# andrewcsmith/soundsym

Hardware: AMD Instinct MI355X
Metric: segment-pairs/sec (DTW cost+argmin) (higher is better)
Workload: dtype f32

## Files before the change

### soundsym_amd/csrc/dtw_filter.hip

```cpp
#include "ssym_internal.hpp"
#include "dtw_filter_kernel.hpp"
#include "dtw_filter_wg_kernel.hpp"
#include "dtw_filter_pk_kernel.hpp"
#include "dtw_filter_sp_kernel.hpp"
#include "dtw_band_kernel.hpp"

#include <algorithm>
#include <atomic>
#include <cmath>
#include <cstdlib>

namespace ssym {

static std::atomic<unsigned long long> g_filter_wg_launches{0};

int filter_pieces(int dim)
{
    static const bool k48 = ssym_knob("SSYM_FILTER_K48") != nullptr;
    return dim > kFilterMaxDim2 ? 1 : (k48 ? 2 : 3);
}

__global__ void build_filter_records_kernel(const double *__restrict__ raw, const uint64_t *__restrict__ off,
                                            const uint32_t *__restrict__ perm, uint32_t n, uint32_t dim,
                                            uint32_t dimUse, uint32_t frames_pad, int is_source,
                                            int lead, int pieces, double scale, _Float16 *__restrict__ rec,
                                            unsigned *__restrict__ resid)
{
    const uint32_t s = blockIdx.y;
    const uint32_t seg = perm[s];
    const uint32_t slot = blockIdx.x * blockDim.x + threadIdx.x;
    if (slot >= frames_pad)
        return;
    _Float16 out[kFilterRecHalfs];
#pragma unroll
    for (int i = 0; i < kFilterRecHalfs; ++i)
        out[i] = (_Float16)0.0f;
    const uint32_t nf = seg < n ? (uint32_t)(off[seg + 1] - off[seg]) : 0u;
    const uint32_t first = lead < 0 ? frames_pad - nf : (uint32_t)lead;
    const bool real = slot >= first && slot < first + nf;
    const uint32_t f = slot - first;
    const int nbase = pieces == 3 ? 28 : (pieces == 2 ? 3 : 1) * (int)dimUse;
    const int npieces = pieces == 3 ? 2 : 3;
    if (!real && is_source)
        out[filter_slot_offset(nbase)] = (_Float16)__builtin_inff();
    if (real) {
        const double *p = raw + (off[seg] + f) * dim;
        double nrm = 0.0, res2 = 0.0;
        for (uint32_t e = 0; e < dimUse; ++e) {
            const double v = p[e] * scale;
            const _Float16 h1 = (_Float16)v;
            const bool two = pieces == 2 || (pieces == 3 && (is_source || e < 2));
            const _Float16 h2 = two ? (_Float16)(v - (double)h1) : (_Float16)0.0f;
            const double vh = (double)h1 + (double)h2;
            nrm += vh * vh;
            res2 += (v - vh) * (v - vh);
            const _Float16 m1 = (_Float16)(-2.0f * (float)h1), m2 = (_Float16)(-2.0f * (float)h2);
            if (pieces == 2) {
                out[filter_slot_offset(3 * e + 0)] = is_source ? m1 : h1;
                out[filter_slot_offset(3 * e + 1)] = is_source ? m1 : h2;
                out[filter_slot_offset(3 * e + 2)] = is_source ? m2 : h1;
            } else if (pieces == 3) {
                out[filter_slot_offset(2 * e + 0)] = is_source ? m1 : h1;
                out[filter_slot_offset(2 * e + 1)] = is_source ? m2 : h1;
                if (e < 2)
                    out[filter_slot_offset(26 + e)] = is_source ? m1 : h2;
            } else {
                out[filter_slot_offset(e)] = is_source ? m1 : h1;
            }
        }
        const float r = __double2float_ru(sqrt(res2) / scale * 1.0000001);
        if (r > 0.0f)
            atomicMax(&resid[s], __float_as_uint(r));
        const _Float16 p1 = (_Float16)nrm;
        const _Float16 p2 = (_Float16)(nrm - (double)p1);
        const _Float16 p3 = (_Float16)(nrm - (double)p1 - (double)p2);
        const int mine = nbase + (is_source ? 0 : npieces), other = nbase + (is_source ? npieces : 0);
        out[filter_slot_offset(mine + 0)] = p1;
        out[filter_slot_offset(mine + 1)] = p2;
        out[filter_slot_offset(other + 0)] = (_Float16)1.0f;
        out[filter_slot_offset(other + 1)] = (_Float16)1.0f;
        if (npieces == 3) {
            out[filter_slot_offset(mine + 2)] = p3;
            out[filter_slot_offset(other + 2)] = (_Float16)1.0f;
        }
    }
    if (is_source) {
        _Float16 *dst = rec + ((size_t)s * frames_pad + slot) * kFilterRecHalfs;
#pragma unroll
        for (int i = 0; i < kFilterRecHalfs; ++i)
            dst[i] = out[i];
    } else {
#pragma unroll
        for (int h = 0; h < 2; ++h)
#pragma unroll
            for (int m = 0; m < kFilterKM; ++m) {
                _Float16 *dst = rec + tgt_rec_offset(s, frames_pad, slot, m, h);
#pragma unroll
                for (int i = 0; i < 8; ++i)
                    dst[i] = out[h * 24 + m * 8 + i];
            }
    }
}

static uint32_t band_slots(int radius, const SegmentSet &src, const SegmentSet &tgt)
{
    const uint32_t kb = (uint32_t)(2 * radius + 1 + 15) / 16 * 16;
    return std::max<uint32_t>(radius + src.max_frames, std::max<uint32_t>(tgt.max_frames, 1) + kb) + 1;
}
static size_t band_lds_bytes(int radius, const SegmentSet &src, const SegmentSet &tgt)
{
    return ((size_t)2 * band_slots(radius, src, tgt) * kFilterRecHalfs + kBandImagePad) * sizeof(_Float16);
}

bool filter_band_as_bound(const ssym_ctx *ctx, const SegmentSet &src, const SegmentSet &tgt)
{
    if (ctx->band < 0)
        return false;
    return 2 * ctx->band + 1 > 6 * 16 || band_lds_bytes(ctx->band, src, tgt) > 160 * 1024 - 64;
}

bool filter_supported(const ssym_ctx *ctx, const SegmentSet &src, const SegmentSet &tgt)
{
    if (src.light || tgt.light)
        return false;
    if (src.dim != tgt.dim)
        return false;
    if ((ctx->band < 0 || filter_band_as_bound(ctx, src, tgt)) && filter_shape((int)src.max_frames).nt == 0)
        return false;
    if (!std::isfinite(src.max_abs) || !std::isfinite(tgt.max_abs))
        return false;
    if (!std::isfinite(src.max_sqnorm_all) || !std::isfinite(tgt.max_sqnorm_all))
        return false;
    return src.n > 0 && tgt.n > 0;
}

static double common_scale(const SegmentSet &src, const SegmentSet &tgt)
{
    const double m = std::max(src.max_abs, tgt.max_abs);
    if (!(m > 0.0))
        return 1.0;
    int e = 0;
    (void)std::frexp(m, &e);
    e = std::min(std::max(6 - e, -100), 100);
    const double sq = std::max(src.max_sqnorm_all, tgt.max_sqnorm_all);
    while (e > -200 && sq * std::ldexp(1.0, 2 * e) * 1.01 >= 65000.0)
        --e;
    const double ideal = std::ldexp(1.0, e);
    if (src.rec && src.rec_scale > 0.0 && src.rec_scale <= ideal && src.rec_scale * 16.0 >= ideal)
        return src.rec_scale;
    return ideal;
}

static int32_t ensure_records(ssym_ctx *ctx, const SegmentSet &set, double scale, uint32_t slots, int lead)
{
    const size_t bytes = (size_t)set.n_pad * slots * kFilterRecHalfs * sizeof(_Float16);
    if (set.rec && set.rec_scale == scale && set.rec_bytes == bytes && set.rec_slots == slots &&
        set.rec_lead == lead)
        return SSYM_OK;
    if (set.rec && set.rec_bytes != bytes) {
        dev_free(ctx, set.rec);
        set.rec = nullptr;
    }
    if (!set.rec) {
        int32_t rca = dev_alloc(ctx, &set.rec, bytes);
        if (rca != SSYM_OK)
            return rca;
    }
    set.rec_bytes = bytes;
    dim3 grid((slots + 63) / 64, set.n_pad);
    const int dimUse = filter_dim_used((int)set.dim);
    unsigned *resid = (unsigned *)(set.max_sqnorm + 2 * (size_t)set.n_pad);
    SSYM_HIP_CHECK(ctx, hipMemsetAsync(resid, 0, sizeof(unsigned) * set.n_pad, ctx->stream));
    build_filter_records_kernel<<<grid, 64, 0, ctx->stream>>>(set.raw, set.off, set.perm, set.n, set.dim,
                                                              (uint32_t)dimUse, slots, set.is_source ? 1 : 0, lead,
                                                              filter_pieces(dimUse), scale,
                                                              (_Float16 *)set.rec, resid);
    SSYM_HIP_CHECK(ctx, hipGetLastError());
    set.rec_scale = scale;
    set.rec_slots = slots;
    set.rec_lead = lead;
    return SSYM_OK;
}

static FilterKnobs read_filter_knobs()
{
    FilterKnobs k;
    if (!ssym_knob("SSYM_TEST_HOOKS"))
        return k;
    auto num = [](const char *name, int unset) {
        const char *v = ssym_knob(name);
        return v ? atoi(v) : unset;
    };
    k.pk = num("SSYM_FILTER_PK", 0) != 0;
    k.sp = num("SSYM_FILTER_SP", 1) != 0;
    const int mp = num("SSYM_SP_MULTIPAIR", 1);
    k.spMultipair = mp == 0 || mp == 2 ? mp : 1;
    k.spPairBlock = ssym_knob("SSYM_SP_PAIRBLOCK") ? std::max(num("SSYM_SP_PAIRBLOCK", 0), 0) : -1;
    k.wg = num("SSYM_FILTER_WG", k.wg) != 0;
    k.skip0 = num("SSYM_FILTER_SKIP0", 1) != 0;
    k.nt8 = ssym_knob("SSYM_FILTER_NT8") != nullptr;
    k.oneLaunch = ssym_knob("SSYM_FILTER_ONE_LAUNCH") != nullptr;
    k.longClasses = num("SSYM_FILTER_LONG_CLASSES", 1) != 0;
    k.pruneNt = num("SSYM_PRUNE_NT", 0);
    return k;
}

static const std::vector<uint32_t> &plan_lens(const SegmentSet &set, uint32_t group)
{
    if (set.plan_lens.size() != set.n_pad / group) {
        set.plan_lens.assign(set.n_pad / group, 0u);
        for (uint32_t slot = 0; slot < set.n; ++slot) {
            const uint32_t s = set.h_perm[slot];
            uint32_t &m = set.plan_lens[slot / group];
            m = std::max(m, (uint32_t)(set.h_off[s + 1] - set.h_off[s]));
        }
    }
    return set.plan_lens;
}

struct FilterCall {
    hipStream_t st;
    const SegmentSet &src, &tgt;
    bool sq;
    int ku;
    float outScale;
    float *handoff;
    unsigned *taskCtr;
    float *cmat;
    const float *abandon;
    unsigned long long *colCtr;
    const uint32_t *candSlot;
};

template <int NT, bool SQ, int KU>
static bool run_kernel(const FilterCall &c, const FilterLaunch &l)
{
    constexpr int OCC = NT == 1 ? 3 : NT == 8 ? 1 : 2;
    const dim3 grid(l.grid), block(64 * kFilterWavesPerBlock);
    const _Float16 *srec = (const _Float16 *)c.src.rec, *trec = (const _Float16 *)c.tgt.rec;
    const int rowsPad = (int)c.src.frames_pad, colsPad = (int)c.tgt.frames_pad, tgtPad = (int)c.tgt.n_pad;
    const int nSrcPairs = l.hi - l.lo, nTasks = nSrcPairs * (tgtPad / 32);
    unsigned *ctr = c.taskCtr + l.ctrSet * 8 * kTaskCtrStride;
    switch (l.kind) {
    case FilterKernel::Mp:
        if constexpr (NT == 1) {
            dtw_filter_sp_kernel<KU == 2 ? 3 : 2, SQ, 2, KU, kSpRowBlock, true><<<grid, block, 0, c.st>>>(
                srec, trec, c.src.len, c.tgt.len, rowsPad, colsPad, tgtPad, l.taskPairs, nSrcPairs, l.taskChunk, c.outScale,
                ctr, c.cmat, l.origin, l.lo, l.pairBlock);
            return true;
        }
        return false;
    case FilterKernel::Sp:
        if constexpr (NT <= 3 && (KU == 2 || NT <= 2)) {
            constexpr int OCCSP = (NT == 1 && KU == 2) ? 3 : (NT == 2 && KU == 2) ? SSYM_SP_OCC_NT2 : 2;
            dtw_filter_sp_kernel<NT, SQ, OCCSP, KU, kSpRowBlock><<<grid, block, 0, c.st>>>(
                srec, trec, c.src.len, c.tgt.len, rowsPad, colsPad, tgtPad, nSrcPairs, nTasks, l.taskChunk, c.outScale, ctr,
                c.cmat, l.origin, l.lo, l.pairBlock);
            return true;
        }
        return false;
    case FilterKernel::GenericSkip0:
        if constexpr (NT == 3 || NT == 4) {
            dtw_filter_kernel<NT, SQ, OCC, false, KU, true><<<grid, block, 0, c.st>>>(
                srec, trec, c.src.len, c.tgt.len, rowsPad, l.passes, colsPad, tgtPad, nSrcPairs, nTasks, l.taskChunk,
                c.outScale, c.handoff, ctr, c.cmat, nullptr, nullptr, nullptr, l.origin, l.lo);
            return true;
        }
        return false;
    case FilterKernel::Wg:
        if constexpr (NT == 4) {
            dtw_filter_wg_kernel<SQ, KU><<<grid, block, 0, c.st>>>(
                srec, trec, c.src.len, c.tgt.len, rowsPad, l.passes, colsPad, tgtPad, nSrcPairs / 4, l.taskChunk, c.outScale,
                c.handoff, ctr, c.cmat, l.origin, l.lo);
            g_filter_wg_launches.fetch_add(1, std::memory_order_relaxed);
            return true;
        }
        return false;
    case FilterKernel::Pk:
        if constexpr (NT == 4) {
            dtw_filter_pk_kernel<SQ, KU><<<grid, block, 0, c.st>>>(
                srec, trec, c.src.len, c.tgt.len, rowsPad, l.passes, colsPad, tgtPad, nSrcPairs, nTasks, l.taskChunk,
                c.outScale, c.handoff, ctr, c.cmat, l.origin, l.lo);
            return true;
        }
        return false;
    case FilterKernel::GenericPrune:
        dtw_filter_kernel<NT, SQ, OCC, true, KU><<<grid, block, 0, c.st>>>(
            srec, trec, c.src.len, c.tgt.len, rowsPad, l.passes, colsPad, tgtPad, nSrcPairs, nTasks, l.taskChunk, c.outScale,
            c.handoff, ctr, c.cmat, c.abandon, c.colCtr, c.candSlot, l.origin, l.lo);
        return true;
    case FilterKernel::Generic:
        dtw_filter_kernel<NT, SQ, OCC, false, KU><<<grid, block, 0, c.st>>>(
            srec, trec, c.src.len, c.tgt.len, rowsPad, l.passes, colsPad, tgtPad, nSrcPairs, nTasks, l.taskChunk, c.outScale,
            c.handoff, ctr, c.cmat, nullptr, nullptr, nullptr, l.origin, l.lo);
        return true;
    }
    return false;
}

template <int NT>
static bool run_tiles(const FilterCall &c, const FilterLaunch &l)
{
    if (c.sq)
        return c.ku == 2 ? run_kernel<NT, true, 2>(c, l) : run_kernel<NT, true, 3>(c, l);
    return c.ku == 2 ? run_kernel<NT, false, 2>(c, l) : run_kernel<NT, false, 3>(c, l);
}

static bool run_launch(const FilterCall &c, const FilterLaunch &l)
{
    switch (l.nt) {
    case 1: return run_tiles<1>(c, l);
    case 2: return run_tiles<2>(c, l);
    case 3: return run_tiles<3>(c, l);
    case 4: return run_tiles<4>(c, l);
    case 8: return run_tiles<8>(c, l);
    }
    return false;
}

template <int NTB, int WB, int OCC, bool SQ, int LASTN, bool PRUNE>
static int32_t launch_band_cfg2(ssym_ctx *ctx, const SegmentSet &src, const SegmentSet &tgt, uint32_t slots,
                                size_t lds, float outScale, float *cmat, const float *abandon,
                                unsigned long long *colCtr, const uint32_t *candSlot)
{
    const int nTgtBlocks = (int)tgt.n_pad / (32 * WB);
    const int nTasks = ((int)src.n_pad / 2) * nTgtBlocks;
    const int grid = std::max(1, std::min(ctx->num_cus, nTasks));
    int32_t rc = ensure(ctx, ctx->handoff, 8 * sizeof(unsigned));
    if (rc != SSYM_OK)
        return rc;
    unsigned *taskCtr = (unsigned *)ctx->handoff.ptr;
    rc = zero_words(ctx, taskCtr, sizeof(unsigned));
    if (rc != SSYM_OK)
        return rc;
    const bool two = filter_mfmas(filter_pieces(filter_dim_used((int)src.dim)), filter_dim_used((int)src.dim)) == 2;
    auto kern = two ? dtw_band_kernel<NTB, WB, OCC, SQ, LASTN, PRUNE, 2> : dtw_band_kernel<NTB, WB, OCC, SQ, LASTN, PRUNE, 3>;
#ifdef SSYM_BAND_PAIRCOLS_BUILD
    if constexpr (!PRUNE && LASTN == 1 && NTB >= 4 && OCC == 2) {
        const char *pc = ssym_knob("SSYM_BAND_PAIRCOLS");
        if (pc && atoi(pc) != 0)
            kern = two ? dtw_band_kernel<NTB, WB, OCC, SQ, LASTN, PRUNE, 2, true> : dtw_band_kernel<NTB, WB, OCC, SQ, LASTN, PRUNE, 3, true>;
    }
#endif
    if (lds > 64 * 1024)
        SSYM_HIP_CHECK(ctx, hipFuncSetAttribute((const void *)kern, hipFuncAttributeMaxDynamicSharedMemorySize, (int)lds));
    kern<<<dim3(grid), 64 * WB, lds, ctx->stream>>>(
        (const _Float16 *)src.rec, (const _Float16 *)tgt.rec, src.len, tgt.len, (int)slots, ctx->band,
        (int)tgt.frames_pad, (int)tgt.n_pad, nTgtBlocks, nTasks, taskCtr, outScale, cmat, abandon, colCtr, candSlot);
    SSYM_HIP_CHECK(ctx, hipGetLastError());
    return SSYM_OK;
}

template <int NTB, int WB, int OCC, bool SQ, int LASTN>
static int32_t launch_band_cfg(ssym_ctx *ctx, const SegmentSet &src, const SegmentSet &tgt, uint32_t slots,
                               size_t lds, float outScale, float *cmat, const float *abandon,
                               unsigned long long *colCtr, const uint32_t *candSlot)
{
    return abandon ? launch_band_cfg2<NTB, WB, OCC, SQ, LASTN, true>(ctx, src, tgt, slots, lds, outScale, cmat, abandon, colCtr, candSlot)
                   : launch_band_cfg2<NTB, WB, OCC, SQ, LASTN, false>(ctx, src, tgt, slots, lds, outScale, cmat, nullptr, nullptr, nullptr);
}

template <int NTB, bool SQ>
static int32_t launch_band(ssym_ctx *ctx, const SegmentSet &src, const SegmentSet &tgt, uint32_t slots,
                           size_t lds, float outScale, float *cmat, const float *abandon, unsigned long long *colCtr, const uint32_t *candSlot)
{
    const bool last1 = 2 * ctx->band + 1 == 16 * (NTB - 1) + 1;
    if constexpr (NTB <= 5)
        return last1 ? launch_band_cfg<NTB, 8, 2, SQ, 1>(ctx, src, tgt, slots, lds, outScale, cmat, abandon, colCtr, candSlot)
                     : launch_band_cfg<NTB, 8, 2, SQ, 16>(ctx, src, tgt, slots, lds, outScale, cmat, abandon, colCtr, candSlot);
    else
        return last1 ? launch_band_cfg<NTB, 4, 1, SQ, 1>(ctx, src, tgt, slots, lds, outScale, cmat, abandon, colCtr, candSlot)
                     : launch_band_cfg<NTB, 4, 1, SQ, 16>(ctx, src, tgt, slots, lds, outScale, cmat, abandon, colCtr, candSlot);
}

static int32_t launch_dtw_filter_banded(ssym_ctx *ctx, const SegmentSet &src, const SegmentSet &tgt, float *cmat,
                                        const float *abandon, unsigned long long *colCtr, const uint32_t *candSlot)
{
    if (tgt.n_pad % kBandTgtQuantum != 0 || src.n_pad % 2 != 0) {
        ctx->err = "dtw band filter: segment set not padded for the banded kernel";
        return SSYM_E_UNSUPPORTED;
    }
    const uint32_t slots = band_slots(ctx->band, src, tgt);
    const size_t lds = band_lds_bytes(ctx->band, src, tgt);
    const double scale = common_scale(src, tgt);
    int32_t rc = ensure_records(ctx, src, scale, slots, ctx->band);
    if (rc != SSYM_OK)
        return rc;
    rc = ensure_records(ctx, tgt, scale, tgt.frames_pad, 0);
    if (rc != SSYM_OK)
        return rc;
    const bool sq = ctx->squared != 0;
    const float outScale = (float)(sq ? 1.0 / (scale * scale) : 1.0 / scale);
    const int ntb = (2 * ctx->band + 1 + 15) / 16;
#define SSYM_BCASE(N_)                                                                                  \
    case N_:                                                                                            \
        return sq ? launch_band<N_, true>(ctx, src, tgt, slots, lds, outScale, cmat, abandon, colCtr, candSlot)   \
                  : launch_band<N_, false>(ctx, src, tgt, slots, lds, outScale, cmat, abandon, colCtr, candSlot);
    switch (ntb) {
        SSYM_BCASE(1) SSYM_BCASE(2) SSYM_BCASE(3) SSYM_BCASE(4) SSYM_BCASE(5) SSYM_BCASE(6)
    default:
        ctx->err = "dtw band filter: band radius too large";
        return SSYM_E_UNSUPPORTED;
    }
#undef SSYM_BCASE
}

int32_t ensure_filter_records(ssym_ctx *ctx, const SegmentSet &src, const SegmentSet &tgt, double *scale_out)
{
    const double scale = common_scale(src, tgt);
    int32_t rc = ctx->band >= 0 && !filter_band_as_bound(ctx, src, tgt)
                     ? ensure_records(ctx, src, scale, band_slots(ctx->band, src, tgt), ctx->band)
                     : ensure_records(ctx, src, scale, src.frames_pad, -1);
    if (rc == SSYM_OK)
        rc = ensure_records(ctx, tgt, scale, tgt.frames_pad, 0);
    if (scale_out)
        *scale_out = scale;
    return rc;
}

int32_t launch_dtw_filter(ssym_ctx *ctx, const SegmentSet &src, const SegmentSet &tgt, float *cmat,
                          const float *abandon, unsigned long long *colCtr, const uint32_t *candSlot)
{
    ctx->filter_launches = 1;
    if (ctx->band >= 0 && !filter_band_as_bound(ctx, src, tgt))
        return launch_dtw_filter_banded(ctx, src, tgt, cmat, abandon, colCtr, candSlot);
    const FilterShape shape = filter_shape((int)src.max_frames);
    if (shape.nt == 0 || (int)src.frames_pad != shape.rows() || src.n_pad % 8 != 0 || tgt.n_pad % 32 != 0) {
        ctx->err = "dtw filter: segment set not padded for the filter kernel";
        return SSYM_E_UNSUPPORTED;
    }
    if (((size_t)tgt.frames_pad + 3) / 4 * 1024 >= ((size_t)1 << 31)) {
        ctx->err = "dtw filter: targets too long for the hand-off rows";
        return SSYM_E_UNSUPPORTED;
    }
    const double scale = common_scale(src, tgt);
    int32_t rc = ensure_records(ctx, src, scale, src.frames_pad, -1);
    if (rc != SSYM_OK)
        return rc;
    rc = ensure_records(ctx, tgt, scale, tgt.frames_pad, 0);
    if (rc != SSYM_OK)
        return rc;
    const int gridBlocks = std::max(8, ctx->num_cus * 2 / 8 * 8);
    const size_t handBytes = (size_t)(gridBlocks / 2 * 3) * kFilterWavesPerBlock * ((tgt.frames_pad + 3) / 4) * 256 * sizeof(float);
    const size_t ctrBytes = 8 * kTaskCtrStride * sizeof(unsigned);
    rc = ensure(ctx, ctx->handoff, handBytes + kMaxClasses * ctrBytes);
    if (rc != SSYM_OK)
        return rc;
    unsigned *taskCtr = (unsigned *)((char *)ctx->handoff.ptr + handBytes);
    rc = zero_words(ctx, taskCtr, kMaxClasses * ctrBytes);
    if (rc != SSYM_OK)
        return rc;
    const bool sq = ctx->squared != 0;
    const int dimUse = filter_dim_used((int)src.dim);

    FilterPlanInput in;
    in.pairLen = plan_lens(src, 2).data(), in.groupCols = plan_lens(tgt, 32).data();
    in.srcN = src.n, in.srcNPad = src.n_pad, in.framesPad = src.frames_pad;
    in.tgtN = tgt.n, in.tgtGroups = tgt.n_pad / 32, in.tgtTotalFrames = tgt.total_frames;
    in.numCus = ctx->num_cus;
    in.ku = filter_mfmas(filter_pieces(dimUse), dimUse);
    in.abandon = abandon != nullptr;
    in.pruneSwept = ctx->prune_swept;
    in.knobs = read_filter_knobs();
    const std::vector<FilterLaunch> plan = plan_filter(in);

    ctx->filter_launches = (int)plan.size();
    ctx->launched_cells = 0;
    for (const FilterLaunch &l : plan)
        ctx->launched_cells += l.cells;
    const FilterCall call{ctx->stream, src, tgt, sq, in.ku, (float)(sq ? 1.0 / (scale * scale) : 1.0 / scale),
                          (float *)ctx->handoff.ptr, taskCtr, cmat, abandon, colCtr, candSlot};
    for (const FilterLaunch &l : plan)
        if (!run_launch(call, l)) {
            ctx->err = "dtw filter: the plan names a kernel that is not built";
            return SSYM_E_UNSUPPORTED;
        }
    SSYM_HIP_CHECK(ctx, hipGetLastError());
    return SSYM_OK;
}

}

extern "C" __attribute__((visibility("default"))) unsigned long long ssym_debug_filter_wg_launches(void)
{
    return ssym::g_filter_wg_launches.load(std::memory_order_relaxed);
}

#ifdef SSYM_SP_PROF
extern "C" __attribute__((visibility("default"))) int ssym_debug_sp_prof(unsigned long long *out)
{
    unsigned long long zero[12] = {0, 0, 0, 0, 0, 0, 0, 0, 0, 0, 0, 0};
    if (hipMemcpyFromSymbol(out, HIP_SYMBOL(ssym::ssym_sp_prof), sizeof(zero)) != hipSuccess)
        return -1;
    return hipMemcpyToSymbol(HIP_SYMBOL(ssym::ssym_sp_prof), zero, sizeof(zero)) == hipSuccess ? 0 : -1;
}
#endif
```

### soundsym_amd/csrc/dtw_filter_wg_kernel.hpp

```cpp
#pragma once
#include "dtw_filter_kernel.hpp"

namespace ssym {

#define SSYM_FILTER_SBASE(P_) asm volatile("" : "+s"(P_))
#define SSYM_FILTER_LANEOFF(V_) asm volatile("" : "+v"(V_))

constexpr int kFilterWgRing = 16;
constexpr int kFilterWgLds = kFilterWgRing * kFilterSlotBytes + kFilterWavesPerBlock * kFilterTopBytes;

template <bool SQ, int KU>
__global__ __launch_bounds__(64 * kFilterWavesPerBlock, 2) void dtw_filter_wg_kernel(
    const _Float16 *__restrict__ srcRec, const _Float16 *__restrict__ tgtRec,
    const int *__restrict__ srcLen, const int *__restrict__ tgtLen, int srcRows, int nPasses,
    int tgtFramesPad, int mPad, int nSrcBlocks, int taskChunk, float outScale,
    float *__restrict__ handoff, unsigned *__restrict__ taskCtr, float *__restrict__ cmat,
    int rowOrigin, int spBase)
{
    static_assert(KU == 2 || KU == 3, "two or three operand planes per column");
    static_assert(kFilterWavesPerBlock == 4, "a column group is one column per wave");
    constexpr int NT = 4;
    constexpr int REC = kFilterRecHalfs;
    constexpr int BR = NT * 16;
    const float INF = __builtin_inff();

    const int lane = threadIdx.x & 63;
    const int wave = __builtin_amdgcn_readfirstlane(threadIdx.x >> 6);
    const int col = lane & 31;
    const int half = lane >> 5;
    const size_t handGroups = ((size_t)tgtFramesPad + 3) / 4;
    char *const handRow = reinterpret_cast<char *>(handoff + ((size_t)blockIdx.x * kFilterWavesPerBlock + wave) * handGroups * 256);
    uint32_t laneOff16 = lane * 16;
    const __amdgpu_buffer_rsrc_t handBuf = __builtin_amdgcn_make_buffer_rsrc(handRow, 0, (int)(handGroups * 1024), 0x00020000);
    constexpr int kWaitStaged = wait_vmcnt(KU), kWaitStagedStores = wait_vmcnt(KU + 4);
    __shared__ __attribute__((aligned(16))) char lds[kFilterWgLds];
    char *const ring = lds;
    char *const myTop = lds + kFilterWgRing * kFilterSlotBytes + wave * kFilterTopBytes;
    volatile unsigned *const taskWord = reinterpret_cast<volatile unsigned *>(lds + kFilterWgRing * kFilterSlotBytes);
    unsigned fetches = 0;

    const unsigned nGroups = (unsigned)mPad >> 5;
    for (unsigned hop = 0; hop < 8; ++hop) {
      const unsigned xcd = (blockIdx.x + hop) & 7u;
      const unsigned rangeLen = xcd < nGroups ? ((nGroups - xcd + 7u) >> 3) * (unsigned)nSrcBlocks : 0u;
      for (;;) {
        if (wave == 0) {
            __builtin_amdgcn_s_waitcnt(wait_vmcnt(0));
            asm volatile("" ::: "memory");
            if (lane == 0)
                taskWord[fetches & 1u] = atomicAdd(&taskCtr[xcd * kTaskCtrStride], (unsigned)taskChunk);
        }
        __syncthreads();
        const unsigned got = (unsigned)__builtin_amdgcn_readfirstlane((int)taskWord[fetches & 1u]);
        ++fetches;
        if (got >= rangeLen)
            break;
        const unsigned gotEnd = min(got + (unsigned)taskChunk, rangeLen);
        int preFa = 0, preFb = 0;
        bool havePre = false;
       for (unsigned gi = got; gi < gotEnd; ++gi) {
        const unsigned lin = rangeLen - 1u - gi;
        const int tg = (int)(xcd + 8u * (lin / (unsigned)nSrcBlocks));
        const int sp = spBase + 4 * (int)(lin % (unsigned)nSrcBlocks) + wave;

        const int fa = havePre ? preFa : srcLen[2 * sp + half];
        const int fb_m1 = (havePre ? preFb : tgtLen[32 * tg + col]) - 1;
        havePre = gi + 1 < gotEnd;
        if (havePre) {
            const unsigned linN = lin - 1u;
            preFa = srcLen[2 * (spBase + 4 * (int)(linN % (unsigned)nSrcBlocks) + wave) + half];
            preFb = tgtLen[32 * (int)(xcd + 8u * (linN / (unsigned)nSrcBlocks)) + col];
        }
        const int r0 = srcRows - fa;

        int nCols = fb_m1 + 1;
#pragma unroll
        for (int o = 32; o >= 1; o >>= 1)
            nCols = max(nCols, __shfl_xor(nCols, o));
        nCols = __builtin_amdgcn_readfirstlane(nCols);

        float res = INF;
        const char *const tgtGroup = reinterpret_cast<const char *>(tgtRec) + (size_t)tg * tgtFramesPad * (kTgtFrameHalfs * 2);

        for (int pass = nCols > 0 ? 0 : nPasses; pass < nPasses; ++pass) {
            const int rowBase = rowOrigin + pass * BR;
            int haveTop = pass, passesLeft = nPasses - 1 - pass;
            asm volatile("" : "+s"(haveTop), "+s"(passesLeft));

            auto stage = [&](int gr) {
                const int c = 4 * gr + wave;
                const int cc = min(c, nCols - 1);
                char *slot = ring + (c & (kFilterWgRing - 1)) * kFilterSlotBytes;
                const char *gb = tgtGroup + (size_t)(unsigned)cc * (kTgtFrameHalfs * 2);
                SSYM_FILTER_SBASE(gb);
                SSYM_FILTER_LANEOFF(laneOff16);
                const __attribute__((address_space(1))) void *gp =
                    (const __attribute__((address_space(1))) void *)(gb + laneOff16);
                __attribute__((address_space(3))) void *lp = (__attribute__((address_space(3))) void *)slot;
                __builtin_amdgcn_global_load_lds(gp, lp, 16, 0, 0);
                __builtin_amdgcn_global_load_lds(gp, lp, 16, 1024, 0);
                if (KU == 3)
                    __builtin_amdgcn_global_load_lds(gp, lp, 16, 2048, 0);
            };
            auto stageTop = [&](int g) {
                const int gg = min(g, (nCols - 1) >> 2);
                __builtin_amdgcn_raw_ptr_buffer_load_lds(handBuf, (__attribute__((address_space(3))) void *)(myTop + (g & 1) * 1024),
                                                         16, laneOff16, gg * 1024, 0, 0);
            };
            auto fetch = [&](int c, half8 (&B)[KU], float &top) {
                const char *slot = ring + (c & (kFilterWgRing - 1)) * kFilterSlotBytes;
#pragma unroll
                for (int m = 0; m < KU; ++m)
                    B[m] = *reinterpret_cast<const half8 *>(slot + m * 1024 + lane * 16);
                top = *reinterpret_cast<const float *>(myTop + ((c >> 2) & 1) * 1024 + (c & 3) * 256 + lane * 4);
            };
            half8 A[NT][KU];
            {
                const int arow = lane & 31;
                const int a_src = 2 * sp + ((arow >> 2) & 1);
                const int a_frm = rowBase + (arow & 3) + 4 * (arow >> 3);
                const _Float16 *abase = srcRec + ((size_t)a_src * srcRows + a_frm) * REC + half * 24;
#pragma unroll
                for (int T = 0; T < NT; ++T)
                    load_rec<KU>(abase + (size_t)T * kFilterRowsPerTile * REC, A[T]);
            }

            asm volatile("" ::: "memory");
            __builtin_amdgcn_s_barrier();
            asm volatile("" ::: "memory");
            if (haveTop)
                stageTop(0);
            stage(0);
            stage(1);

            float L0[BR], L1[BR];
#pragma unroll
            for (int i = 0; i < BR; ++i) {
                L0[i] = (rowBase + i == r0 - 1) ? 0.0f : INF;
                L1[i] = L0[i];
            }
            float prevTop = (rowBase == r0) ? 0.0f : INF;

            half8 B0[KU], B1[KU];
            float topN = INF;
            __builtin_amdgcn_s_waitcnt(kWaitStaged);
            asm volatile("" ::: "memory");
            if (!haveTop) {
                typedef float f32x4 __attribute__((ext_vector_type(4)));
                *reinterpret_cast<f32x4 *>(myTop + lane * 16) = f32x4{INF, INF, INF, INF};
                *reinterpret_cast<f32x4 *>(myTop + 1024 + lane * 16) = f32x4{INF, INF, INF, INF};
            }
            __builtin_amdgcn_s_barrier();
            asm volatile("" ::: "memory");
            fetch(0, B0, topN);
            f32x16 acc = mfma_tile<KU>(A[0], B0);

            for (int j0 = 0; j0 < nCols; j0 += 4) {
                const int g = j0 >> 2;
                stage(g + 2);
                SSYM_FILTER_SBASE(passesLeft);
                if (passesLeft == 0 || j0 == 0)
                    __builtin_amdgcn_s_waitcnt(kWaitStaged);
                else
                    __builtin_amdgcn_s_waitcnt(kWaitStagedStores);
                asm volatile("" ::: "memory");
                __builtin_amdgcn_s_barrier();
                asm volatile("" ::: "memory");
#pragma unroll
                for (int q = 0; q < 4; ++q) {
                    const int j = j0 + q;
                    if (j < nCols) {
                        const float up = topN;
                        const float diag = prevTop;
                        prevTop = up;
                        SSYM_FILTER_SBASE(haveTop);
                        SSYM_FILTER_SBASE(passesLeft);
                        if (q == 3 && haveTop) {
                            if (passesLeft == 0)
                                __builtin_amdgcn_s_waitcnt(wait_vmcnt(0));
                            else
                                __builtin_amdgcn_s_waitcnt(wait_vmcnt(3));
                            asm volatile("" ::: "memory");
                        }
                        if ((q & 1) == 0)
                            fetch(j + 1, B1, topN);
                        else
                            fetch(j + 1, B0, topN);
                        if (q == 0 && haveTop)
                            stageTop(g + 1);
                        float bottom;
                        if ((q & 1) == 0)
                            bottom = dp_column<NT, SQ, KU>(A, B0, B1, acc, up, diag, L0, L1);
                        else
                            bottom = dp_column<NT, SQ, KU>(A, B1, B0, acc, up, diag, L1, L0);
                        SSYM_FILTER_SBASE(passesLeft);
                        if (passesLeft != 0) {
                            __builtin_amdgcn_raw_buffer_store_b32(__float_as_uint(bottom), handBuf, lane * 4, g * 1024 + q * 256, 0);
                        } else {
                            res = (j == fb_m1) ? bottom : res;
                        }
                    }
                }
            }
        }
        cmat[(size_t)(2 * sp + half) * mPad + 32 * tg + col] = res * outScale;
       }
      }
    }
}

#undef SSYM_FILTER_SBASE
#undef SSYM_FILTER_LANEOFF

}
```

Measured before the change: 512.0 million.

## Add two-pass workgroup DTW filter kernel with leader/follower waves via LDS handoff

Adds a new wg2 kernel for two-pass workgroup filter launches. Leader waves compute the top row band and pass each column's bottom value to follower waves through LDS, and the followers compute the second band concurrently in a tick-synchronised pipeline. This replaces the sequential two passes that handed off through a global buffer. A front-end task fetcher and a shared target-staging ring are interleaved into the ticks. The kernel is enabled by default, adds per-tick barriers, and halves the pairs processed per block. An ablation macro is also added to the old kernel.

```diff
diff --git a/soundsym_amd/csrc/dtw_filter.hip b/soundsym_amd/csrc/dtw_filter.hip
--- a/soundsym_amd/csrc/dtw_filter.hip
+++ b/soundsym_amd/csrc/dtw_filter.hip
@@ -1,6 +1,7 @@
 #include "ssym_internal.hpp"
 #include "dtw_filter_kernel.hpp"
 #include "dtw_filter_wg_kernel.hpp"
+#include "dtw_filter_wg2_kernel.hpp"
 #include "dtw_filter_pk_kernel.hpp"
 #include "dtw_filter_sp_kernel.hpp"
 #include "dtw_band_kernel.hpp"
@@ -13,6 +14,8 @@
 namespace ssym {
 
 static std::atomic<unsigned long long> g_filter_wg_launches{0};
+static std::atomic<unsigned long long> g_filter_wg2_launches{0};
+static std::atomic<bool> g_filter_wg2{true};
 
 int filter_pieces(int dim)
 {
@@ -185,6 +188,7 @@
 static FilterKnobs read_filter_knobs()
 {
     FilterKnobs k;
+    g_filter_wg2.store(true, std::memory_order_relaxed);
     if (!ssym_knob("SSYM_TEST_HOOKS"))
         return k;
     auto num = [](const char *name, int unset) {
@@ -197,6 +201,7 @@
     k.spMultipair = mp == 0 || mp == 2 ? mp : 1;
     k.spPairBlock = ssym_knob("SSYM_SP_PAIRBLOCK") ? std::max(num("SSYM_SP_PAIRBLOCK", 0), 0) : -1;
     k.wg = num("SSYM_FILTER_WG", k.wg) != 0;
+    g_filter_wg2.store(num("SSYM_FILTER_WG2", 1) != 0, std::memory_order_relaxed);
     k.skip0 = num("SSYM_FILTER_SKIP0", 1) != 0;
     k.nt8 = ssym_knob("SSYM_FILTER_NT8") != nullptr;
     k.oneLaunch = ssym_knob("SSYM_FILTER_ONE_LAUNCH") != nullptr;
@@ -230,6 +235,7 @@
     const float *abandon;
     unsigned long long *colCtr;
     const uint32_t *candSlot;
+    bool wg2;
 };
 
 template <int NT, bool SQ, int KU>
@@ -269,6 +275,14 @@
         return false;
     case FilterKernel::Wg:
         if constexpr (NT == 4) {
+            if (l.passes == 2 && c.wg2) {
+                dtw_filter_wg2_kernel<SQ, KU><<<grid, block, 0, c.st>>>(
+                    srec, trec, c.src.len, c.tgt.len, rowsPad, colsPad, tgtPad, nSrcPairs / 4, l.taskChunk, c.outScale, ctr,
+                    c.cmat, l.origin, l.lo);
+                g_filter_wg_launches.fetch_add(1, std::memory_order_relaxed);
+                g_filter_wg2_launches.fetch_add(1, std::memory_order_relaxed);
+                return true;
+            }
             dtw_filter_wg_kernel<SQ, KU><<<grid, block, 0, c.st>>>(
                 srec, trec, c.src.len, c.tgt.len, rowsPad, l.passes, colsPad, tgtPad, nSrcPairs / 4, l.taskChunk, c.outScale,
                 c.handoff, ctr, c.cmat, l.origin, l.lo);
@@ -469,7 +483,8 @@
     for (const FilterLaunch &l : plan)
         ctx->launched_cells += l.cells;
     const FilterCall call{ctx->stream, src, tgt, sq, in.ku, (float)(sq ? 1.0 / (scale * scale) : 1.0 / scale),
-                          (float *)ctx->handoff.ptr, taskCtr, cmat, abandon, colCtr, candSlot};
+                          (float *)ctx->handoff.ptr, taskCtr, cmat, abandon, colCtr, candSlot,
+                          g_filter_wg2.load(std::memory_order_relaxed)};
     for (const FilterLaunch &l : plan)
         if (!run_launch(call, l)) {
             ctx->err = "dtw filter: the plan names a kernel that is not built";
@@ -486,6 +501,11 @@
     return ssym::g_filter_wg_launches.load(std::memory_order_relaxed);
 }
 
+extern "C" __attribute__((visibility("default"))) unsigned long long ssym_debug_filter_wg2_launches(void)
+{
+    return ssym::g_filter_wg2_launches.load(std::memory_order_relaxed);
+}
+
 #ifdef SSYM_SP_PROF
 extern "C" __attribute__((visibility("default"))) int ssym_debug_sp_prof(unsigned long long *out)
 {
diff --git a/soundsym_amd/csrc/dtw_filter_wg2_kernel.hpp b/soundsym_amd/csrc/dtw_filter_wg2_kernel.hpp
--- /dev/null
+++ b/soundsym_amd/csrc/dtw_filter_wg2_kernel.hpp
@@ -0,0 +1,290 @@
+#pragma once
+#include "dtw_filter_kernel.hpp"
+
+namespace ssym {
+
+#define SSYM_FILTER_SBASE(P_) asm volatile("" : "+s"(P_))
+#define SSYM_FILTER_LANEOFF(V_) asm volatile("" : "+v"(V_))
+
+constexpr int kFilterWg2Ring = 16;
+constexpr int kFilterWg2HandBytes = 2 * 2 * 1024;
+constexpr int kFilterWg2RecBytes = 2 * 16;
+constexpr int kFilterWg2LenBytes = 256;
+constexpr int kFilterWg2Lds = kFilterWg2Ring * kFilterSlotBytes + kFilterWg2HandBytes + kFilterWg2RecBytes + kFilterWg2LenBytes;
+constexpr int wait_vmcnt_lgkm0(int n) { return wait_vmcnt(n) & ~0x0F00; }
+
+template <bool SQ, int KU>
+__global__ __launch_bounds__(64 * kFilterWavesPerBlock, 2) void dtw_filter_wg2_kernel(
+    const _Float16 *__restrict__ srcRec, const _Float16 *__restrict__ tgtRec,
+    const int *__restrict__ srcLen, const int *__restrict__ tgtLen, int srcRows,
+    int tgtFramesPad, int mPad, int nSrcBlocks, int taskChunk, float outScale,
+    unsigned *__restrict__ taskCtr, float *__restrict__ cmat, int rowOrigin, int spBase)
+{
+    static_assert(KU == 2 || KU == 3, "two or three operand planes per column");
+    static_assert(kFilterWavesPerBlock == 4, "two pairs x two roles; a column group is one column per wave");
+    constexpr int NT = 4;
+    constexpr int REC = kFilterRecHalfs;
+    constexpr int BR = NT * 16;
+    const float INF = __builtin_inff();
+
+    const int lane = threadIdx.x & 63;
+    const int wave = __builtin_amdgcn_readfirstlane(threadIdx.x >> 6);
+    const int follower = wave & 1;
+    const int col = lane & 31;
+    const int half = lane >> 5;
+    uint32_t laneOff16 = lane * 16;
+    __shared__ __attribute__((aligned(16))) char lds[kFilterWg2Lds];
+    char *const ring = lds;
+    char *const hand = lds + kFilterWg2Ring * kFilterSlotBytes + (wave >> 1) * 2048;
+    volatile int *const record = reinterpret_cast<volatile int *>(lds + kFilterWg2Ring * kFilterSlotBytes + kFilterWg2HandBytes);
+
+    char *const lenBuf = lds + kFilterWg2Ring * kFilterSlotBytes + kFilterWg2HandBytes + kFilterWg2RecBytes;
+    uint32_t laneOff4 = lane * 4;
+
+    const unsigned nGroups = (unsigned)mPad >> 5;
+
+    struct Item { int tg, sp0, nCols, g; };
+    Item im1{0, 0, 0, -1}, i0{0, 0, 0, -1}, i1{0, 0, 0, -1}, i2{0, 0, 0, -1};
+    unsigned hop = 0;
+    unsigned requests = 0;
+    bool pending = false;
+    bool request = false;
+    unsigned tick = 0;
+    unsigned feGi = 0, feEnd = 0, feHalf = 0, feXcd = 0, feRange = 0;
+    bool feOn = false, feAtomic = false, feValid = false;
+    unsigned feTk = 0;
+    int feTg = 0, feSp0 = 0;
+
+    auto last_group = [](const Item &it) __attribute__((always_inline)) { return 4 * (it.g + 1) >= it.nCols; };
+
+    auto open_tick = [&](bool storeYoungest) __attribute__((always_inline)) -> bool {
+        if (storeYoungest)
+            __builtin_amdgcn_s_waitcnt(wait_vmcnt_lgkm0(1));
+        else
+            __builtin_amdgcn_s_waitcnt(wait_vmcnt_lgkm0(0));
+        asm volatile("" ::: "memory");
+        __builtin_amdgcn_s_barrier();
+        asm volatile("" ::: "memory");
+        im1 = i0;
+        i0 = i1;
+        i1 = i2;
+        if (i2.g >= 0 && !last_group(i2)) {
+            ++i2.g;
+        } else if (pending) {
+            const unsigned slot = (requests - 1u) & 1u;
+            const int tg = __builtin_amdgcn_readfirstlane(record[4 * slot + 0]);
+            const int sp0 = __builtin_amdgcn_readfirstlane(record[4 * slot + 1]);
+            const int nc = __builtin_amdgcn_readfirstlane(record[4 * slot + 2]);
+            if (tg >= 0) {
+                i2 = Item{tg, sp0, nc, 0};
+            } else {
+                i2.g = -1;
+                ++hop;
+            }
+        } else {
+            i2.g = -1;
+        }
+        pending = false;
+        if (hop >= 8u && im1.g < 0 && i0.g < 0 && i1.g < 0 && i2.g < 0)
+            return false;
+        request = hop < 8u && (i2.g < 0 || last_group(i2));
+        if (request) {
+            pending = true;
+            ++requests;
+        }
+        feOn = request && wave == 0;
+        if (feOn) {
+            feXcd = (blockIdx.x + hop) & 7u;
+            feRange = feXcd < nGroups ? ((nGroups - feXcd + 7u) >> 3) * (unsigned)nSrcBlocks : 0u;
+            feAtomic = feGi >= feEnd;
+            if (feAtomic && lane == 0)
+                feTk = atomicAdd(&taskCtr[feXcd * kTaskCtrStride], (unsigned)taskChunk);
+        }
+        if (i2.g >= 0) {
+            const int cc = max(min(4 * i2.g + wave, i2.nCols - 1), 0);
+            char *slot = ring + ((4 * (tick + 2u) + (unsigned)wave) & (unsigned)(kFilterWg2Ring - 1)) * kFilterSlotBytes;
+            const char *gb = reinterpret_cast<const char *>(tgtRec) +
+                             ((size_t)(unsigned)i2.tg * (unsigned)tgtFramesPad + (unsigned)cc) * (kTgtFrameHalfs * 2);
+            SSYM_FILTER_SBASE(gb);
+            SSYM_FILTER_LANEOFF(laneOff16);
+            const __attribute__((address_space(1))) void *gp =
+                (const __attribute__((address_space(1))) void *)(gb + laneOff16);
+            __attribute__((address_space(3))) void *lp = (__attribute__((address_space(3))) void *)slot;
+            __builtin_amdgcn_global_load_lds(gp, lp, 16, 0, 0);
+            __builtin_amdgcn_global_load_lds(gp, lp, 16, 1024, 0);
+            if (KU == 3)
+                __builtin_amdgcn_global_load_lds(gp, lp, 16, 2048, 0);
+        }
+        asm volatile("" ::: "memory");
+        return true;
+    };
+    auto front_end_task = [&]() __attribute__((always_inline)) {
+        if (feOn) {
+            if (feAtomic) {
+                feGi = (unsigned)__builtin_amdgcn_readfirstlane((int)feTk);
+                feEnd = min(feGi + (unsigned)taskChunk, feRange);
+                feHalf = 0;
+            }
+            feValid = feGi < feEnd;
+            if (feValid) {
+                const unsigned lin = feRange - 1u - feGi;
+                feTg = (int)(feXcd + 8u * (lin / (unsigned)nSrcBlocks));
+                feSp0 = spBase + 4 * (int)(lin % (unsigned)nSrcBlocks) + 2 * (int)feHalf;
+                const int *gl = tgtLen + 32 * feTg;
+                SSYM_FILTER_SBASE(gl);
+                SSYM_FILTER_LANEOFF(laneOff4);
+                __builtin_amdgcn_global_load_lds(
+                    (const __attribute__((address_space(1))) void *)(reinterpret_cast<const char *>(gl) + (laneOff4 & 127u)),
+                    (__attribute__((address_space(3))) void *)lenBuf, 4, 0, 0);
+            }
+        }
+    };
+    auto front_end_record = [&]() __attribute__((always_inline)) {
+        if (feOn) {
+            int nc = 0;
+            if (feValid) {
+                __builtin_amdgcn_s_waitcnt(wait_vmcnt(0));
+                asm volatile("" ::: "memory");
+                nc = *reinterpret_cast<volatile int *>(lenBuf + laneOff4);
+#pragma unroll
+                for (int o = 32; o >= 1; o >>= 1)
+                    nc = max(nc, __shfl_xor(nc, o));
+                nc = __builtin_amdgcn_readfirstlane(nc);
+            }
+            const unsigned slot = (requests - 1u) & 1u;
+            if (lane == 0) {
+                record[4 * slot + 0] = feValid ? feTg : -1;
+                record[4 * slot + 1] = feSp0;
+                record[4 * slot + 2] = nc;
+            }
+            if (feValid) {
+                feHalf ^= 1u;
+                if (feHalf == 0)
+                    ++feGi;
+            } else {
+                feGi = feEnd = feHalf = 0;
+            }
+        }
+    };
+    auto fetch = [&](unsigned s, half8 (&B)[KU]) __attribute__((always_inline)) {
+        const char *slot = ring + (s & (unsigned)(kFilterWg2Ring - 1)) * kFilterSlotBytes;
+#pragma unroll
+        for (int m = 0; m < KU; ++m)
+            B[m] = *reinterpret_cast<const half8 *>(slot + m * 1024 + lane * 16);
+    };
+
+    half8 A[NT][KU];
+    float L0[BR], L1[BR];
+    half8 B0[KU], B1[KU];
+    f32x16 acc;
+    float prevTop = INF;
+    auto start_task = [&](const Item &it, int rowBase, unsigned vg) __attribute__((always_inline)) {
+        const int sp = it.sp0 + (wave >> 1);
+        const int fa = srcLen[2 * sp + half];
+        {
+            const int arow = lane & 31;
+            const int a_src = 2 * sp + ((arow >> 2) & 1);
+            const int a_frm = rowBase + (arow & 3) + 4 * (arow >> 3);
+            const _Float16 *abase = srcRec + ((size_t)a_src * srcRows + a_frm) * REC + half * 24;
+#pragma unroll
+            for (int T = 0; T < NT; ++T)
+                load_rec<KU>(abase + (size_t)T * kFilterRowsPerTile * REC, A[T]);
+        }
+        const int r0 = srcRows - fa;
+#pragma unroll
+        for (int i = 0; i < BR; ++i) {
+            L0[i] = (rowBase + i == r0 - 1) ? 0.0f : INF;
+            L1[i] = L0[i];
+        }
+        prevTop = (rowBase == r0) ? 0.0f : INF;
+        fetch(4u * vg, B0);
+        acc = mfma_tile<KU>(A[0], B0);
+    };
+
+    if (!follower) {
+        float up = INF;
+        asm volatile("" : "+v"(up));
+        for (;; ++tick) {
+            if (!open_tick(false))
+                break;
+            if (i0.g >= 0) {
+                const unsigned vg = tick & 3u;
+                if (i0.g == 0)
+                    start_task(i0, rowOrigin, vg);
+                char *const handW = hand + (tick & 1u) * 1024 + lane * 4;
+                auto column = [&](int q) __attribute__((always_inline)) {
+                    const float diag = prevTop;
+                    prevTop = up;
+                    float bottom;
+                    if ((q & 1) == 0) {
+                        fetch(4u * vg + q + 1, B1);
+                        bottom = dp_column<NT, SQ, KU>(A, B0, B1, acc, up, diag, L0, L1);
+                    } else {
+                        fetch(4u * vg + q + 1, B0);
+                        bottom = dp_column<NT, SQ, KU>(A, B1, B0, acc, up, diag, L1, L0);
+                    }
+                    *reinterpret_cast<float *>(handW + q * 256) = bottom;
+                };
+                column(0);
+                column(1);
+                front_end_task();
+                column(2);
+                column(3);
+                front_end_record();
+            } else {
+                front_end_task();
+                front_end_record();
+            }
+        }
+    } else {
+        float res = INF;
+        int fb_m1 = -1;
+        bool stored = false;
+        for (;; ++tick) {
+            if (!open_tick(stored))
+                break;
+            stored = false;
+            if (im1.g >= 0) {
+                const unsigned vg = (tick + 3u) & 3u;
+                const char *const handR = hand + ((tick + 1u) & 1u) * 1024 + lane * 4;
+                float topN = *reinterpret_cast<const float *>(handR);
+                if (im1.g == 0) {
+                    fb_m1 = tgtLen[32 * im1.tg + col] - 1;
+                    res = INF;
+                    start_task(im1, rowOrigin + BR, vg);
+                }
+                const int j0 = 4 * im1.g;
+                auto column = [&](int q) __attribute__((always_inline)) {
+                    const float up = topN;
+                    const float diag = prevTop;
+                    prevTop = up;
+                    if (q < 3)
+                        topN = *reinterpret_cast<const float *>(handR + (q + 1) * 256);
+                    float bottom;
+                    if ((q & 1) == 0) {
+                        fetch(4u * vg + q + 1, B1);
+                        bottom = dp_column<NT, SQ, KU>(A, B0, B1, acc, up, diag, L0, L1);
+                    } else {
+                        fetch(4u * vg + q + 1, B0);
+                        bottom = dp_column<NT, SQ, KU>(A, B1, B0, acc, up, diag, L1, L0);
+                    }
+                    res = (j0 + q == fb_m1) ? bottom : res;
+                };
+                column(0);
+                column(1);
+                column(2);
+                column(3);
+                if (last_group(im1)) {
+                    const int sp = im1.sp0 + (wave >> 1);
+                    cmat[(size_t)(2 * sp + half) * mPad + 32 * im1.tg + col] = res * outScale;
+                    stored = true;
+                }
+            }
+        }
+    }
+}
+
+#undef SSYM_FILTER_SBASE
+#undef SSYM_FILTER_LANEOFF
+
+}
diff --git a/soundsym_amd/csrc/dtw_filter_wg_kernel.hpp b/soundsym_amd/csrc/dtw_filter_wg_kernel.hpp
--- a/soundsym_amd/csrc/dtw_filter_wg_kernel.hpp
+++ b/soundsym_amd/csrc/dtw_filter_wg_kernel.hpp
@@ -84,7 +84,11 @@
 
         for (int pass = nCols > 0 ? 0 : nPasses; pass < nPasses; ++pass) {
             const int rowBase = rowOrigin + pass * BR;
+#ifdef SSYM_ABL_NOHAND
+            int haveTop = 0, passesLeft = nPasses - 1 - pass;
+#else
             int haveTop = pass, passesLeft = nPasses - 1 - pass;
+#endif
             asm volatile("" : "+s"(haveTop), "+s"(passesLeft));
 
             auto stage = [&](int gr) {
@@ -195,7 +199,11 @@
                             bottom = dp_column<NT, SQ, KU>(A, B1, B0, acc, up, diag, L1, L0);
                         SSYM_FILTER_SBASE(passesLeft);
                         if (passesLeft != 0) {
+#ifndef SSYM_ABL_NOHAND
                             __builtin_amdgcn_raw_buffer_store_b32(__float_as_uint(bottom), handBuf, lane * 4, g * 1024 + q * 256, 0);
+#else
+                            res = (j == fb_m1 - 1) ? bottom : res;
+#endif
                         } else {
                             res = (j == fb_m1) ? bottom : res;
                         }
```

Result: faster. 530.3 million (median of 6 runs) (+3.6%).
